# anhtu293/nndepth

Hardware: AMD Instinct MI355X
Metric: stereo pairs/sec at 544x960, 32 iters (RAFT-Stereo) (higher is better)
Workload: dtype f32 carried as 2 range-scaled fp16 pieces per operand (3 MFMA products, fp32 accumulate)

## Files before the change

### nndepth_amd/csrc/common.h

```cpp
#pragma once
#include <hip/hip_runtime.h>
#include <atomic>
#include <cstdarg>
#include <cstdio>
#include "../../include/nndepth_amd.h"

namespace nnd {

void set_error(const char* fmt, ...);

#define NND_HIP_CHECK(expr)                                                              \
    do {                                                                                 \
        hipError_t _e = (expr);                                                          \
        if (_e != hipSuccess) {                                                          \
            nnd::set_error("%s failed: %s (%s:%d)", #expr, hipGetErrorString(_e), __FILE__, __LINE__); \
            return NND_ERR_HIP;                                                          \
        }                                                                                \
    } while (0)

#define NND_LAUNCH_CHECK()                                                               \
    do {                                                                                 \
        hipError_t _e = hipGetLastError();                                               \
        if (_e != hipSuccess) {                                                          \
            nnd::set_error("kernel launch failed: %s (%s:%d)", hipGetErrorString(_e), __FILE__, __LINE__); \
            return NND_ERR_HIP;                                                          \
        }                                                                                \
    } while (0)

#define NND_REQUIRE(cond, ...)                                                           \
    do {                                                                                 \
        if (!(cond)) {                                                                   \
            nnd::set_error(__VA_ARGS__);                                                 \
            return NND_ERR_INVALID;                                                      \
        }                                                                                \
    } while (0)

struct Switches {
    bool no_fused_upsample, no_fused_lookup, no_fused_flow_branch, no_c4, agcl_v1, no_thin3d, corr_build_v1, corr_build_no_ksplit, igev_squeeze_v1, igev_squeeze_walk, no_folded_flow_head, no_conv1x1_stream,
        conv_verbose, debug_sync;
    int split_ny, split_ks, split_p;
    bool split_no_fast;
    bool no_merged_fb_lookup;
    int conv_p, conv_ks, conv_wco;
    int agcl_pb;
    bool lds_poison_on;
    unsigned lds_poison;
    int lds_slack;
    bool enc_no_c4;
    bool no_slab3d;
    int slab3d_rounds;
};
const Switches& switches();

static inline int raise_lds_limit(const void* kern, std::atomic<unsigned>& done, int bytes = 160 * 1024) {
    int dev = 0;
    NND_HIP_CHECK(hipGetDevice(&dev));
    const unsigned bit = 1u << (dev & 31);
    if (!(done.load(std::memory_order_relaxed) & bit)) {
        NND_HIP_CHECK(hipFuncSetAttribute(kern, hipFuncAttributeMaxDynamicSharedMemorySize, bytes));
        done.fetch_or(bit, std::memory_order_relaxed);
    }
    return NND_OK;
}

bool calibrating();
struct CalibScope {
    explicit CalibScope(bool on);
// ... 115 lines not shown
int lookup_convc1_launch(const float* pyr, const float* geo, int G, const float* coords, const ConvLayer& L, const float* blob,
                         float* c1, int64_t c1_bs, int B, int H, int W, int num_levels, int radius, hipStream_t stream, bool c1_c4);
bool flow_branch_lookup_supported(int arith);
int flow_branch_lookup_launch(const ConvLayer& f2, const float* blob, const float* w7t, const float* b7, const float* flow, int64_t fbs,
                              int fc, const ConvIO& io, const float* pyr, const float* coords, const ConvLayer& Lc1, float* c1,
                              int64_t c1_bs, int B, int H, int W, int num_levels, int radius, hipStream_t stream, bool c1_c4);
bool igev_lookup_convc1_il_supported(int G, int num_levels, int radius);
int igev_lookup_convc1_il_launch(const float* il, int G, const float* coords, const ConvLayer& L, const float* blob, float* c1,
                                 int64_t c1_bs, int B, int H, int W, int num_levels, int radius, hipStream_t stream, bool c1_c4);
struct MaskUpFlowHead {
    const float* x;
    long xbs;
    int hid;
    const float* w;
    const float* bias;
    const float* coords_in;
    float *coords_out, *flow_out, *delta_out;
    float* hx_flow;
    long hx_bs;
    int hx_pm;
    int absolute;
};

bool mask_upsample_supported(int rate, int cin, int flow_channels);
bool mask_upsample_fold_supported(const ConvLayer& L, int hid);
int mask_upsample_launch(const ConvLayer& L, const float* blob, const float* x, int64_t xbs, const float* flow, float* out,
                         int B, int H, int W, int rate, hipStream_t stream, bool tiled, int flow_channels = 1, bool x_c4 = false,
                         const MaskUpFlowHead* fh = nullptr);

}
```

### nndepth_amd/csrc/error.cpp

```cpp
#include "common.h"

#include <cstdlib>

namespace nnd {
static thread_local char g_err[512] = "";
void set_error(const char* fmt, ...) {
    va_list ap;
    va_start(ap, fmt);
    vsnprintf(g_err, sizeof(g_err), fmt, ap);
    va_end(ap);
}

static Switches g_sw;
static void load_switches() {
    Switches s{};
    auto on = [](const char* n) { return getenv(n) != nullptr; };
    s.no_fused_upsample = on("NND_NO_FUSED_UPSAMPLE");
    s.no_fused_lookup = on("NND_NO_FUSED_LOOKUP");
    s.no_fused_flow_branch = on("NND_NO_FUSED_FLOW_BRANCH");
    s.no_c4 = on("NND_NO_C4");
    s.agcl_v1 = on("NND_AGCL_V1");
    s.no_thin3d = on("NND_NO_THIN3D");
    s.corr_build_v1 = on("NND_CORR_BUILD_V1");
    s.corr_build_no_ksplit = on("NND_CORR_BUILD_NO_KSPLIT");
    s.igev_squeeze_v1 = on("NND_IGEV_SQUEEZE_V1");
    s.igev_squeeze_walk = on("NND_IGEV_SQUEEZE_WALK");
    s.no_folded_flow_head = on("NND_NO_FOLDED_FLOW_HEAD");
    s.no_conv1x1_stream = on("NND_NO_CONV1X1_STREAM");
    s.conv_verbose = on("NND_CONV_VERBOSE");
    s.debug_sync = on("NND_DEBUG_SYNC");
    s.split_ny = s.split_ks = s.split_p = -1;
    if (const char* e = getenv("NND_SPLIT_CFG")) sscanf(e, "%d,%d,%d", &s.split_ny, &s.split_ks, &s.split_p);
    s.split_no_fast = on("NND_SPLIT_NO_FAST");
    s.no_merged_fb_lookup = on("NND_NO_MERGED_FB_LOOKUP");
    s.conv_p = s.conv_ks = s.conv_wco = -1;
    if (const char* e = getenv("NND_CONV_CFG")) sscanf(e, "%d,%d,%d", &s.conv_p, &s.conv_ks, &s.conv_wco);
    if (const char* e = getenv("NND_CONV_P")) s.conv_p = atoi(e);
    s.agcl_pb = getenv("NND_AGCL_PB") ? atoi(getenv("NND_AGCL_PB")) : 0;
    s.lds_poison_on = on("NND_DEBUG_LDS_POISON");
    s.lds_poison = s.lds_poison_on ? (unsigned)strtoul(getenv("NND_DEBUG_LDS_POISON"), nullptr, 0) : 0u;
    s.lds_slack = getenv("NND_DEBUG_LDS_SLACK") ? atoi(getenv("NND_DEBUG_LDS_SLACK")) : 0;
    s.enc_no_c4 = on("NND_ENC_NO_C4");
    s.no_slab3d = on("NND_NO_SLAB3D");
    s.slab3d_rounds = getenv("NND_SLAB3D_ROUNDS") ? atoi(getenv("NND_SLAB3D_ROUNDS")) : 0;
    g_sw = s;
}
namespace {
struct SwitchInit {
    SwitchInit() { load_switches(); }
} g_switch_init;
// ... 21 lines not shown
```

### nndepth_amd/csrc/mask_upsample.hip

```cpp
#include "common.h"

#include <type_traits>
#include "layout.h"
#include "split_arith.h"

namespace nnd {

typedef float f32x16 __attribute__((ext_vector_type(16)));

#ifdef NND_DBG_STAMPS
__device__ unsigned long long g_mu_stamps[4096 * 8];
#define NND_MSTAMP(i)                                                                             \
    do {                                                                                          \
        if (threadIdx.x == 0 && blockIdx.x < 4096) g_mu_stamps[blockIdx.x * 8 + (i)] = __builtin_amdgcn_s_memrealtime(); \
    } while (0)
#else
#define NND_MSTAMP(i)
#endif

struct MaskUpArgs {
    const float* x;
    long xbs;
    const float* wpk;
    const float* bias;
    const float* flow;
    float* out;
    int H, W, tiles_x, fc;
    Lay lay;
    int x_c4;
    int lds_floats;
    MaskUpFlowHead fh;
};

template <int RATE, int CIN>
struct MaskUpCfg {
    static constexpr int COUT = 9 * RATE * RATE;
    static constexpr int NCB = (COUT + 31) / 32;
    static constexpr int CBW = NCB >= 12 ? 3 : 1;
    static constexpr int G = (NCB + CBW - 1) / CBW;
    static constexpr int NWAVES = 2 * G;
    static constexpr int NT = 64 * NWAVES;
    static constexpr int NST = CIN / 32;
    static constexpr int MT_STRIDE = 33;
    static constexpr int XS_FLOATS = CIN * 32 * 3 / 2;
    static constexpr int LDS_FLOATS = (XS_FLOATS > COUT * MT_STRIDE ? XS_FLOATS : COUT * MT_STRIDE) + 128;
};

template <int RATE, int CIN, int NS = 0, int FHW = 0>
__global__ void __launch_bounds__((MaskUpCfg<RATE, CIN>::NT + 64 * FHW)) mask_upsample_kernel(MaskUpArgs a) {
    constexpr bool SPLIT = NS != 0;
    using Cfg = MaskUpCfg<RATE, CIN>;
    constexpr int COUT = Cfg::COUT, NCB = Cfg::NCB, CBW = Cfg::CBW, G = Cfg::G, NT = Cfg::NT, NST = Cfg::NST;
    constexpr int CI_T = 128;
    constexpr int NCHUNK = CIN / CI_T;
    constexpr int MTS = Cfg::MT_STRIDE;
    static_assert(CIN % 128 == 0 && NST % 2 == 0, "CIN must be a multiple of 128");
    extern __shared__ float lds[];
    NND_MSTAMP(0);
    float* xs = lds;
    float* mt = lds;
    float* fp = lds + a.lds_floats - 128;

    const int tid = threadIdx.x, lane = tid & 63;
    const int wave = __builtin_amdgcn_readfirstlane(tid >> 6);
    const int g = wave % G, kj = wave / G;
    const int h2 = lane >> 5, l31 = lane & 31;
    const int tx0 = (blockIdx.x % a.tiles_x) * 8, ty0 = (blockIdx.x / a.tiles_x) * 4;
    const int b = blockIdx.z;
    const int H = a.H, W = a.W;
    const long HW = (long)H * W;
    const long XP = a.lay.plane;
    float oscale = 1.f, xscale = 1.f;
    if constexpr (NS == 2) {
        oscale = a.bias[Cfg::NCB * 32 + SPLIT_TAIL_OSCALE];
        xscale = a.bias[Cfg::NCB * 32 + SPLIT_TAIL_XSCALE];
    }

    float fh_state = 0.f, fh_bias = 0.f;
    auto fh_finish = [&](float* fbase, int t0) {
        if (t0 >= 60) return;
        const float* part = fbase + a.fh.hid * 105;
        const int pr = t0 / 10, pc = t0 % 10;
        const int y = ty0 + pr - 1, x = tx0 + pc - 1;
        float sum = 0.f;
#pragma unroll
        for (int sl = 0; sl < 16; ++sl) sum += part[sl * 64 + t0];
        sum += fh_bias;
        const bool in = y >= 0 && y < H && x >= 0 && x < W;
        const float cnew = fh_state + sum;
        const float fl = a.fh.absolute ? cnew : cnew - (float)x;
        fp[t0] = in ? fl : 0.f;
        if (in && pr >= 1 && pr <= 4 && pc >= 1 && pc <= 8) {
            const long pix = pix_off(a.lay, y, x);
            a.fh.delta_out[b * XP + pix] = sum;
            a.fh.coords_out[b * XP + pix] = cnew;
            a.fh.flow_out[b * XP + pix] = fl;
            a.fh.hx_flow[b * a.fh.hx_bs + pix * a.fh.hx_pm] = fl;
        }
    };
    constexpr int NQ4 = (CIN / 4 * 32 + NT - 1) / NT;
    float4 v4[SPLIT ? NQ4 : 1];
    if constexpr (SPLIT) {
        const float* src = a.x + b * a.xbs;
#pragma unroll
        for (int i = 0; i < NQ4; ++i) {
            const int e = min(tid, NT - 1) + i * NT;
            const int qd = e >> 5, px = e & 31;
            const int y = ty0 + (px >> 3), x = tx0 + (px & 7);
            const bool ok = e < CIN / 4 * 32 && y < H && x < W;
            if (a.x_c4) {
                v4[i] = *reinterpret_cast<const float4*>(src + (ok ? (unsigned)(qd * 4 * (int)XP + 4 * (int)pix_off(a.lay, y, x)) : 0u));
            } else {
                const unsigned o = ok ? (unsigned)(qd * 4 * (int)XP + (int)pix_off(a.lay, y, x)) : 0u;
                v4[i] = make_float4(src[o], src[ok ? o + (unsigned)XP : 0u], src[ok ? o + 2u * (unsigned)XP : 0u], src[ok ? o + 3u * (unsigned)XP : 0u]);
            }
        }
    }
    if constexpr (FHW > 0) {
        if (tid >= NT) {
            float* fbase = lds + Cfg::LDS_FLOATS;
            const int hid = a.fh.hid, fw_ = __builtin_amdgcn_readfirstlane((tid - NT) >> 6), cn = hid / FHW, c0 = fw_ * cn;
            float* patch = fbase;
            float* fw = fbase + hid * 96;
            const float* src = a.fh.x + b * a.fh.xbs;
            constexpr int NPL = 12, NWL = 5;
            const int total = 96 * (cn / 4), nwt = cn * 9;
            float4 pv[NPL];
            bool pok[NPL];
            float wreg[NWL];
#pragma unroll
            for (int k = 0; k < NWL; ++k) wreg[k] = a.fh.w[c0 * 9 + min(lane + 64 * k, nwt - 1)];
            if (tid - NT < 60) {
                fh_bias = a.fh.bias[0];
                const int y = ty0 + (tid - NT) / 10 - 1, x = tx0 + (tid - NT) % 10 - 1;
                if (y >= 0 && y < H && x >= 0 && x < W) fh_state = a.fh.coords_in[b * XP + pix_off(a.lay, y, x)];
            }
#pragma unroll
// ... 43 lines not shown
#pragma unroll
                        for (int t = 0; t < 9; ++t) wv[k][t] = wk[t];
                    }
#pragma unroll
                    for (int k = 0; k < 4; ++k)
#pragma unroll
                        for (int t = 0; t < 9; ++t) fmac_scalar(acc[k], wv[k][t], xv[k][t]);
                }
                float* part = fbase + hid * 105;
                if (lane < 60)
#pragma unroll
                    for (int k = 0; k < 4; ++k) part[(s0 + k) * 64 + pos] = acc[k];
            }
            __syncthreads();
            fh_finish(fbase, tid - NT);
            __syncthreads();
            __syncthreads();
            return;
        }
    }
    {
        const float* src = a.x + b * a.xbs;
        if constexpr (SPLIT) {
            unsigned char* xsb = reinterpret_cast<unsigned char*>(lds);
#pragma unroll
            for (int i = 0; i < NQ4; ++i) {
                const int e = tid + i * NT;
                const int qd = e >> 5, px = e & 31;
                const bool ok = (ty0 + (px >> 3)) < H && (tx0 + (px & 7)) < W;
                if (e < CIN / 4 * 32) {
                    const float res[4] = {ok ? v4[i].x : 0.f, ok ? v4[i].y : 0.f, ok ? v4[i].z : 0.f, ok ? v4[i].w : 0.f};
                    const int chunk = qd >> 2, sub = qd & 3;
                    constexpr int NP = NS == 0 ? 3 : NS;
                    uint2 pv[NP];
                    split_pieces_n<NP, 4, uint2>(res, pv, xscale);
#pragma unroll
                    for (int sp = 0; sp < NP; ++sp)
                        *reinterpret_cast<uint2*>(xsb + ((((chunk * NP + sp) * 2 + (sub >> 1)) * 32 + px) * 16 + (sub & 1) * 8)) = pv[sp];
                }
            }
        } else
        if (a.x_c4) {
            constexpr int NQ4 = (CIN / 4 * 32 + NT - 1) / NT;
            float4 v4[NQ4];
#pragma unroll
            for (int i = 0; i < NQ4; ++i) {
                const int e = tid + i * NT;
                const int qd = e >> 5, px = e & 31;
                const int y = ty0 + (px >> 3), x = tx0 + (px & 7);
                const bool ok = e < CIN / 4 * 32 && y < H && x < W;
                v4[i] = *reinterpret_cast<const float4*>(src + (ok ? (unsigned)(qd * 4 * (int)XP + 4 * (int)pix_off(a.lay, y, x)) : 0u));
            }
#pragma unroll
            for (int i = 0; i < NQ4; ++i) {
// ... 9 lines not shown
            }
        } else {
        constexpr int NLD = (CIN * 32 + NT - 1) / NT;
        float v[NLD];
#pragma unroll
        for (int i = 0; i < NLD; ++i) {
            const int e = tid + i * NT;
            const int ci = e >> 5, px = e & 31;
            const int y = ty0 + (px >> 3), x = tx0 + (px & 7);
            const bool ok = e < CIN * 32 && y < H && x < W;
            v[i] = src[ok ? (unsigned)(ci * (int)XP + (int)pix_off(a.lay, y, x)) : 0u];
        }
#pragma unroll
        for (int i = 0; i < NLD; ++i) {
            const int e = tid + i * NT;
            const int px = e & 31;
            const bool ok = (ty0 + (px >> 3)) < H && (tx0 + (px & 7)) < W;
            if (e < CIN * 32) xs[e] = ok ? v[i] : 0.f;
        }
        }
        if (!a.fh.x && tid < 60 * a.fc) {
            const int f = tid / 60, pos = tid % 60;
            const int pr = pos / 10, pc = pos % 10;
            const int y = ty0 + pr - 1, x = tx0 + pc - 1;
            fp[tid] = (y >= 0 && y < H && x >= 0 && x < W) ? a.flow[(b * a.fc + f) * XP + pix_off(a.lay, y, x)] : 0.f;
        }
    }
    __syncthreads();
    NND_MSTAMP(1);

    f32x16 acc[CBW];
#pragma unroll
    for (int i = 0; i < CBW; ++i)
#pragma unroll
        for (int r = 0; r < 16; ++r) acc[i][r] = 0.f;
    if constexpr (SPLIT) {
        constexpr int NP = NS == 0 ? 3 : NS;
        constexpr int NCH16 = CIN / 16, CPW = NCH16 / 2;
        const uint4* wq4 = reinterpret_cast<const uint4*>(a.wpk);
        const unsigned char* xsb = reinterpret_cast<const unsigned char*>(lds);
        const int c0k = kj * CPW;
        auto a_ptr = [&](int cbi, int ch) {
            int cb = g * CBW + cbi;
            cb = cb < NCB ? cb : NCB - 1;
            return wq4 + (size_t)((cb * NCH16 + c0k + ch) * NP) * 64 + lane;
        };
        constexpr int AD = 3, NA = AD + 1, NUNIT = CPW * CBW;
        uint4 ab[NA][NP], bq[2][NP];
        auto load_a = [&](uint4* dst, int u) {
            const uint4* w = a_ptr(u % CBW, u / CBW);
#pragma unroll
            for (int sp = 0; sp < NP; ++sp) dst[sp] = w[sp * 64];
        };
        auto load_b = [&](uint4* dst, int ch) {
#pragma unroll
            for (int sp = 0; sp < NP; ++sp)
                dst[sp] = *reinterpret_cast<const uint4*>(xsb + (((((c0k + ch) * NP + sp) * 2 + h2) * 32 + l31) * 16));
        };
#pragma unroll
        for (int u = 0; u < AD && u < NUNIT; ++u) load_a(ab[u], u);
        load_b(bq[0], 0);
#pragma unroll
        for (int u = 0; u < NUNIT; ++u) {
            const int ch = u / CBW, cbi = u % CBW;
            if (u + AD < NUNIT) load_a(ab[(u + AD) % NA], u + AD);
            if (cbi == 0 && ch + 1 < CPW) load_b(bq[(ch + 1) & 1], ch + 1);
            __builtin_amdgcn_sched_barrier(0);
            split_mfma_step<NP>(ab[u % NA], bq[ch & 1], acc[cbi]);
            __builtin_amdgcn_sched_barrier(0);
        }
        if constexpr (NS == 2) {
#pragma unroll
            for (int cbi = 0; cbi < CBW; ++cbi)
#pragma unroll
                for (int r = 0; r < 16; ++r) acc[cbi][r] *= oscale;
        }
    } else {
        constexpr int SPW = NST / 2;
        const int s0 = kj * SPW;
        const float4* wq = reinterpret_cast<const float4*>(a.wpk);
        auto a_base = [&](int cbi) {
            int cb = g * CBW + cbi;
            cb = cb < NCB ? cb : NCB - 1;
            return wq + (size_t)cb * (NCHUNK * 16 * 64);
        };
        float4 ab[2][4];
        float bq[2][16];
        auto load_a = [&](float4* dst, int u) {
            const int s = s0 + u / CBW, cbi = u % CBW;
            const float4* ws = a_base(cbi) + s * (4 * 64);
    #pragma unroll
            for (int q = 0; q < 4; ++q) dst[q] = ws[(unsigned)(q * 64 + lane)];
        };
        auto load_b = [&](float* dst, int sl) {
            const float* xb = xs + ((s0 + sl) * 32 + h2) * 32 + l31;
    #pragma unroll
            for (int pair = 0; pair < 16; ++pair) dst[pair] = xb[pair * 64];
        };
        load_a(ab[0], 0);
        load_b(bq[0], 0);
    #pragma unroll
        for (int u = 0; u < SPW * CBW; ++u) {
            const int sl = u / CBW, cbi = u % CBW;
            if (u + 1 < SPW * CBW) load_a(ab[(u + 1) & 1], u + 1);
            if (cbi == 0 && sl + 1 < SPW) load_b(bq[(sl + 1) & 1], sl + 1);
            __builtin_amdgcn_sched_barrier(0);
    #pragma unroll
            for (int pair = 0; pair < 16; ++pair) {
                const float4 av = ab[u & 1][pair / 4];
                const float as = (pair % 4 == 0) ? av.x : (pair % 4 == 1) ? av.y : (pair % 4 == 2) ? av.z : av.w;
                acc[cbi] = __builtin_amdgcn_mfma_f32_32x32x2f32(as, bq[sl & 1][pair], acc[cbi], 0, 0, 0);
            }
            __builtin_amdgcn_sched_barrier(0);
        }
}
    NND_MSTAMP(2);
    __syncthreads();

#pragma unroll
    for (int pass = 0; pass < 2; ++pass) {
        if (kj == pass) {
#pragma unroll
            for (int cbi = 0; cbi < CBW; ++cbi) {
                const int cb = g * CBW + cbi;
#pragma unroll
                for (int reg = 0; reg < 16; ++reg) {
                    const int co = cb * 32 + (reg & 3) + 8 * (reg >> 2) + 4 * h2;
                    if (cb < NCB && co < COUT) {
                        float* p = mt + co * MTS + l31;
                        *p = pass == 0 ? acc[cbi][reg] : *p + acc[cbi][reg];
                    }
                }
            }
        }
        __syncthreads();
    }

    NND_MSTAMP(3);
    constexpr int ROWLEN = 8 * RATE;
    constexpr int NITEM = 4 * RATE * ROWLEN;
    const long OW = (long)W * RATE;
    for (int e = tid; e < NITEM; e += NT) {
        const int seg = e / ROWLEN, within = e % ROWLEN;
        const int rr = seg / RATE, i = seg % RATE;
        const int c = within / RATE, j = within % RATE;
        const int px = rr * 8 + c;
        const int y = ty0 + rr, x = tx0 + c;
        float m[9];
        float mx = -INFINITY;
#pragma unroll
        for (int k = 0; k < 9; ++k) {
            const int co = k * RATE * RATE + i * RATE + j;
            m[k] = 0.25f * (mt[co * MTS + px] + a.bias[co]);
            mx = fmaxf(mx, m[k]);
        }
        float sum = 0.f;
#pragma unroll
        for (int k = 0; k < 9; ++k) {
            m[k] = expf(m[k] - mx);
            sum += m[k];
        }
#pragma unroll
        for (int k = 0; k < 9; ++k) m[k] = m[k] / sum;
        for (int f = 0; f < a.fc; ++f) {
            float o = 0.f;
#pragma unroll
            for (int k = 0; k < 9; ++k) o += m[k] * ((float)RATE * fp[f * 60 + (rr + k / 3) * 10 + c + k % 3]);
            if (y < H && x < W) a.out[((long)b * a.fc + f) * HW * RATE * RATE + ((long)y * RATE + i) * OW + (long)x * RATE + j] = o;
        }
    }
#ifdef NND_DBG_STAMPS
    __builtin_amdgcn_s_waitcnt(0);
#endif
    NND_MSTAMP(4);
}

constexpr int MU_FHW = 4;
template <int RATE, int CIN, int NS, int FHW>
static int launch_mu_fhw(MaskUpArgs a, int B, hipStream_t stream) {
    using Cfg = MaskUpCfg<RATE, CIN>;
    auto kern = mask_upsample_kernel<RATE, CIN, NS, FHW>;
    a.lds_floats = Cfg::LDS_FLOATS;
    const int fh_floats = a.fh.x ? a.fh.hid * (96 + 9) + 16 * 64 : 0;
    if (FHW > 0) a.lds_floats = Cfg::LDS_FLOATS + fh_floats + 128;
    const size_t lds = a.lds_floats * sizeof(float);
    if (lds > 64 * 1024) {
        static std::atomic<unsigned> raised{0};
        if (int rc = raise_lds_limit(reinterpret_cast<const void*>(kern), raised)) return rc;
    }
    dim3 grid(a.tiles_x * cdiv(a.H, 4), 1, B), block(Cfg::NT + 64 * FHW);
    hipLaunchKernelGGL(kern, grid, block, lds, stream, a);
    NND_LAUNCH_CHECK();
    return NND_OK;
}
template <int RATE, int CIN, int NS = 0>
static int launch_mu(const MaskUpArgs& a, int B, hipStream_t stream) {
    if (a.fh.x) {
        if constexpr (NS == 2) return launch_mu_fhw<RATE, CIN, NS, MU_FHW>(a, B, stream);
        else NND_REQUIRE(false, "mask_upsample: the folded flow head is built for the fp16x2 arithmetic");
    }
    return launch_mu_fhw<RATE, CIN, NS, 0>(a, B, stream);
}

bool mask_upsample_fold_supported(const ConvLayer& L, int hid) { return L.arith == 2 && hid % 16 == 0 && hid <= 128; }

bool mask_upsample_supported(int rate, int cin, int flow_channels) {
    return (flow_channels == 1 || flow_channels == 2) && ((rate == 8 && (cin == 256 || cin == 128)) || (rate == 4 && (cin == 256 || cin == 128)));
}

int mask_upsample_launch(const ConvLayer& L, const float* blob, const float* x, int64_t xbs, const float* flow, float* out,
                         int B, int H, int W, int rate, hipStream_t stream, bool tiled, int flow_channels, bool x_c4,
                         const MaskUpFlowHead* fh) {
    NND_REQUIRE(L.KH == 1 && L.KW == 1 && L.CI_T == (L.arith ? 16 : 128) && L.Cout == 9 * rate * rate && (L.arith == 0 || L.arith == 3 || L.arith == 2),
                "mask_upsample: layer shape / packing");
    NND_REQUIRE(mask_upsample_supported(rate, L.Cin, flow_channels), "mask_upsample: rate %d / Cin %d / %d flow channels not built",
                rate, L.Cin, flow_channels);
    MaskUpArgs a;
    a.x = x; a.xbs = xbs; a.wpk = blob + L.w_off; a.bias = blob + L.b_off; a.flow = flow; a.out = out;
    a.H = H; a.W = W; a.tiles_x = cdiv(W, 8); a.fc = flow_channels;
    a.lay = make_lay(H, W, tiled);
    a.x_c4 = (tiled && x_c4) ? 1 : 0;
    a.lds_floats = 0;
    a.fh = MaskUpFlowHead{};
    if (fh && fh->x) {
        NND_REQUIRE(flow_channels == 1 && mask_upsample_fold_supported(L, fh->hid) && fh->w && fh->bias && fh->coords_in && fh->coords_out && fh->flow_out &&
                        fh->delta_out && fh->hx_flow && fh->coords_in != fh->coords_out,
                    "mask_upsample: folded flow head needs one flow channel, hid %% 16 == 0 and distinct old / new state buffers");
        a.fh = *fh;
    }
    if (L.arith == 3) {
        if (rate == 8 && L.Cin == 256) return launch_mu<8, 256, 3>(a, B, stream);
        if (rate == 8 && L.Cin == 128) return launch_mu<8, 128, 3>(a, B, stream);
        if (rate == 4 && L.Cin == 256) return launch_mu<4, 256, 3>(a, B, stream);
        return launch_mu<4, 128, 3>(a, B, stream);
    }
    if (L.arith == 2) {
        if (calibrating()) {
            const Act xa{const_cast<float*>(x), xbs, L.Cin};
            if (int rc = calib_amax_act(xa, make_lay(H, W, tiled, x_c4), B, H, W, blob + L.tail_off(), stream)) return rc;
        }
        if (rate == 8 && L.Cin == 256) return launch_mu<8, 256, 2>(a, B, stream);
        if (rate == 8 && L.Cin == 128) return launch_mu<8, 128, 2>(a, B, stream);
        if (rate == 4 && L.Cin == 256) return launch_mu<4, 256, 2>(a, B, stream);
        return launch_mu<4, 128, 2>(a, B, stream);
    }
    if (rate == 8 && L.Cin == 256) return launch_mu<8, 256>(a, B, stream);
    if (rate == 8 && L.Cin == 128) return launch_mu<8, 128>(a, B, stream);
    if (rate == 4 && L.Cin == 256) return launch_mu<4, 256>(a, B, stream);
    return launch_mu<4, 128>(a, B, stream);
}

#ifdef NND_DBG_STAMPS
extern "C" int nnd_debug_read_mu_stamps(unsigned long long* host, int n) {
    return hipMemcpyFromSymbol(host, HIP_SYMBOL(g_mu_stamps), sizeof(unsigned long long) * n) == hipSuccess ? 0 : -1;
}
#endif

}
```

### nndepth_amd/csrc/update_block.hip

```cpp
#include "common.h"
#include "layout.h"

#include <cstdlib>
#include <cstring>
#include <vector>

namespace nnd {

enum ConvId { C_C1 = 0, C_C2, C_F2, C_CV, C_ZR1X, C_Q1X, C_ZR2X, C_Q2X, C_FHM, C_M2, C_LOOP_COUNT,
              C_ZR1 = C_LOOP_COUNT, C_Q1, C_ZR2, C_Q2, C_ZR1C, C_Q1C, C_ZR2C, C_Q2C, C_COUNT };
static const char* kConvNames[C_COUNT] = {"encoder.convc1", "encoder.convc2", "encoder.convf2", "encoder.conv",
                                          "gru.convz1+convr1[h,motion]", "gru.convq1[rh,motion]", "gru.convz2+convr2[h,motion]",
                                          "gru.convq2[rh,motion]", "flow_head.conv1+mask.0", "mask.2",
                                          "gru.convz1+convr1", "gru.convq1", "gru.convz2+convr2", "gru.convq2",
                                          "gru.convz1+convr1[inp]", "gru.convq1[inp]", "gru.convz2+convr2[inp]", "gru.convq2[inp]"};

struct Plan {
    nnd_update_block_desc d;
    bool sep;
    ConvLayer L[C_COUNT];
    int64_t f1_w, f1_b;
    int64_t f1_wt;
    int64_t fc2_w, fc2_b;
    int64_t total;
};
// ... 48 lines not shown
        p->L[zr - C_ZR1 + C_ZR1C] = mk(kh, kw, ctx, 2 * hid, &off, ar(zr - C_ZR1 + C_ZR1C));
        p->L[q - C_ZR1 + C_ZR1C] = mk(kh, kw, ctx, hid, &off, ar(q - C_ZR1 + C_ZR1C));
    }
    if (!p->sep)
        for (int base : {(int)C_ZR1X, (int)C_ZR1, (int)C_ZR1C}) {
            p->L[base + 2] = p->L[base];
            p->L[base + 3] = p->L[base + 1];
        }
    p->L[C_FHM] = mk(3, 3, hid, 3 * hid, &off, ar(C_FHM));
    p->fc2_w = off; off += (int64_t)fc * hid * 9;
    p->fc2_b = off; off += 4;
    p->L[C_M2] = mk(1, 1, 2 * hid, mc, &off, ar(C_M2));
    p->total = off;
    return NND_OK;
}

static int refuse_last_only(const nnd_update_block_desc* d, const char* what) {
    NND_REQUIRE(!d || !(d->flags & NND_FLAG_LAST_UPSAMPLE_ONLY), "%s: NND_FLAG_LAST_UPSAMPLE_ONLY applies to the refine entry points only", what);
    return NND_OK;
}

struct Bufs {
    float *c1, *cf, *f1, *hx, *z, *rh, *fm, *corr, *mask, *delta, *coords, *flow, *ctxb;
    int64_t total;
};

static void carve(const Plan& p, int B, int H, int W, float* base, Bufs* b) {
    const int64_t n = (int64_t)B * tiled_plane(H, W);
    const int hid = p.d.hidden_dim, ctx = p.d.context_dim, fc = p.d.flow_channels;
    int64_t off = 0;
    auto take = [&](int C) {
        float* ptr = base ? base + off : nullptr;
        off += ((int64_t)C * n + 63) / 64 * 64;
        return ptr;
    };
    b->c1 = take(256);
    b->cf = take(256);
    b->f1 = take(128);
    b->hx = take(2 * hid + ctx);
    b->z = take(hid);
    b->rh = take(hid);
    b->fm = take(3 * hid);
    b->corr = take(p.d.cor_planes);
    b->mask = take(p.d.mask_channels);
    b->delta = take(fc);
    b->coords = take(1);
    b->flow = take(fc);
    b->ctxb = take(6 * hid);
    b->total = off;
}

template <int FC>
__global__ void __launch_bounds__(256) convf1_kernel(const float* __restrict__ flow, long fbs, const float* __restrict__ w,
                                                     const float* __restrict__ bias, float* __restrict__ out, long obs,
                                                     int H, int W, int tiles_x, Lay lay) {
    __shared__ float patch[FC][14][40];
    __shared__ __attribute__((aligned(16))) float wl[16 * (FC * 49 + 3)];
    constexpr int WS = FC * 49 + 3;
    const int tid = threadIdx.x;
    const int tx0 = (blockIdx.x % tiles_x) * 32, ty0 = (blockIdx.x / tiles_x) * 8;
    const int b = blockIdx.z, co0 = blockIdx.y * 16;
    const long HW = lay.plane;
    for (int e = tid; e < FC * 14 * 38; e += 256) {
        int c = e / (14 * 38), rem = e % (14 * 38);
        int pr = rem / 38, pc = rem % 38;
        int gy = ty0 + pr - 3, gx = tx0 + pc - 3;
        patch[c][pr][pc] = (gy >= 0 && gy < H && gx >= 0 && gx < W) ? flow[b * fbs + c * HW + pix_off(lay, gy, gx)] : 0.f;
    }
    for (int e = tid; e < 16 * FC * 49; e += 256) wl[(e / (FC * 49)) * WS + e % (FC * 49)] = w[(long)co0 * (FC * 49) + e];
    __syncthreads();
    const int st = tid >> 5, within = tid & 31;
// ... 598 lines not shown
                        agcl_offset_cl_supported(cre->C) && !switches().agcl_v1;
    if (cre_cl) {
        NND_TRY(nchw_to_nhwc_launch(cre->f1, cre->warped, B, cre->C, H * W, s));
        NND_TRY(nchw_to_nhwc_launch(cre->f2, cre->warped + (int64_t)B * cre->C * H * W, B, cre->C, H * W, s));
    }
    Act c = act(w.corr, p.d.cor_planes * n, p.d.cor_planes);
    auto lookup = [&](hipStream_t st_, int it) -> int {
        if (cre) {
            if (cre->extra && cre_cl)
                return agcl_offset_cl_launch(cre->warped, cre->warped + (int64_t)B * cre->C * H * W, w.flow, cre->extra, w.corr, B, cre->C,
                                             H, W, it & 1, st_, true);
            if (cre->extra) return agcl_offset_launch(cre->f1, cre->f2, w.flow, cre->extra, w.corr, B, cre->C, H, W, it & 1, st_, true);
            return agcl_iter_launch(cre->f1, cre->f2, w.flow, cre->warped, w.corr, B, cre->C, H, W, it & 1, st_, true);
        }
        if (igev) return igev_lookup_launch(pyramid, geo_pyramid, w.coords, w.corr, B, groups, H, W, num_levels, radius, st_, true);
        if (flat_groups > 0) return group_lookup_flat_launch(pyramid, w.coords, w.corr, B, flat_groups, H, W, num_levels, radius, st_, true);
        return corr1d_lookup_launch(pyramid, w.coords, w.corr, B, H, W, num_levels, radius, st_, true);
    };
    for (int id : {(int)C_ZR1C, (int)C_Q1C, (int)C_ZR2C, (int)C_Q2C})
        if (p.sep || id < C_ZR2C) NND_TRY(run_conv(p, packed, w, id, c, nullptr, nullptr, B, H, W, s));
    const bool no_fuse_up = switches().no_fused_upsample;
    const bool no_fuse_lk = switches().no_fused_lookup;
    const bool fused_up = !no_fuse_up && mask_upsample_supported(rate, 2 * hid, fc);
    const bool fold_fh = fused_up && !cre && fc == 1 && mask_upsample_fold_supported(p.L[C_M2], hid) &&
                         (long)B * cdiv(H, 4) * cdiv(W, 8) <= 256 && !switches().no_folded_flow_head;
    float* coords_alt = w.mask;
    float* flow_alt = w.mask + ((int64_t)B * n + 63) / 64 * 64;
    const bool fused_lk = !cre && !no_fuse_lk && flat_groups == 0;
    const bool merged_fbl = fused_lk && !igev && !switches().no_merged_fb_lookup && !switches().no_fused_flow_branch &&
                            flow_branch_supported(p.L[C_F2], fc) && flow_branch_lookup_supported(p.L[C_F2].arith);
    auto loop_conv = [&](int id) -> int {
        probe_mark(id, s);
        const int rc_ = run_conv(p, packed, w, id, c, nullptr, nullptr, B, H, W, s);
        probe_mark(id, s);
        return rc_;
    };
    if (calibrating() && fused_lk && interleaved && p.L[C_C1].arith == 2 && igev_lookup_convc1_il_supported(groups, num_levels, radius))
        NND_TRY(calib_amax_flat(interleaved, nnd_igev_interleaved_floats(B, groups, H, W, num_levels), packed + p.L[C_C1].tail_off(), s));
    for (int it = 0; it < iters; ++it) {
        if (merged_fbl) {
            probe_mark(C_F2, s);
            NND_TRY(calib_flow_branch(p, packed, w, w.flow, B, H, W, s));
            const ConvIO fio = conv_io(p, w, C_F2, c, n, nullptr, nullptr);
            NND_TRY(flow_branch_lookup_launch(p.L[C_F2], packed, packed + p.f1_wt, packed + p.f1_b, w.flow, (int64_t)fc * n, fc, fio, pyramid,
                                              w.coords, p.L[C_C1], w.c1, 256 * n, B, H, W, num_levels, radius, s, ws_c4()));
            NND_TRY(debug_sync("encoder.convf1+convf2 | lookup+convc1", s));
            probe_mark(C_F2, s);
        } else {
// ... 10 lines not shown
            NND_TRY(debug_sync("lookup+convc1", s));
        } else {
            NND_TRY(lookup(s, it));
            NND_TRY(debug_sync("lookup", s));
            NND_TRY(run_conv(p, packed, w, C_C1, c, nullptr, nullptr, B, H, W, s));
        }
        }
        NND_TRY(loop_conv(C_C2));
        NND_TRY(loop_conv(C_CV));
        NND_TRY(loop_conv(C_ZR1X));
        NND_TRY(loop_conv(C_Q1X));
        if (p.sep) {
            NND_TRY(loop_conv(C_ZR2X));
            NND_TRY(loop_conv(C_Q2X));
        }
        if (last_only && it + 1 < iters) {
            ConvIO io = conv_io(p, w, C_FHM, c, n, nullptr, nullptr);
            io.cout_need = hid;
            NND_TRY(launch_conv(p.L[C_FHM], packed, io, conv_epi(C_FHM), B, H, W, s));
            NND_TRY(debug_sync("flow_head.conv1", s));
            NND_TRY(run_fc2(p, packed, w, w.delta, cre ? 2 : 1, igev, B, H, W, s));
            continue;
        }
        NND_TRY(loop_conv(C_FHM));
        float* up_it = up_out + (int64_t)it * up_iter_stride;
        if (fold_fh) {
            MaskUpFlowHead fh;
            fh.x = w.fm; fh.xbs = (int64_t)3 * hid * n; fh.hid = hid;
            fh.w = packed + p.fc2_w; fh.bias = packed + p.fc2_b;
            fh.coords_in = w.coords; fh.coords_out = coords_alt; fh.flow_out = flow_alt; fh.delta_out = w.delta;
            fh.hx_flow = hx_flow; fh.hx_bs = (long)(hxC * n); fh.hx_pm = ws_pm(); fh.absolute = igev ? 1 : 0;
            NND_TRY(mask_upsample_launch(p.L[C_M2], packed, w.fm + hid * n, (int64_t)3 * hid * n, w.flow, up_it, B, H, W, rate, s,
                                         true, fc, ws_c4(), &fh));
            NND_TRY(debug_sync("flow_head.conv2 + mask.2 + upsample", s));
            std::swap(w.coords, coords_alt);
            std::swap(w.flow, flow_alt);
            continue;
        }
        NND_TRY(run_fc2(p, packed, w, w.delta, cre ? 2 : 1, igev, B, H, W, s));
        if (fused_up) {
            NND_TRY(mask_upsample_launch(p.L[C_M2], packed, w.fm + hid * n, (int64_t)3 * hid * n, w.flow, up_it, B, H, W, rate, s,
                                         true, fc, ws_c4()));
            NND_TRY(debug_sync("mask.2 + upsample", s));
        } else {
            NND_TRY(run_conv(p, packed, w, C_M2, c, w.mask, nullptr, B, H, W, s));
            NND_TRY(convex_upsample_launch(w.flow, w.mask, up_it, B, fc, H, W, rate, s, true));
            NND_TRY(debug_sync("convex upsample", s));
        }
// ... 345 lines not shown
```

Baseline: 148.2.

## Defer mask upsampling and batch several iterations into one launch

Keeps a ring of per-iteration hidden-state and flow buffers and launches the convex mask upsample once per group of iterations, covering all grouped slots in one grid. It also lets one workgroup process two tiles so each weight load feeds MFMAs for both. This targets the small, poorly occupied per-iteration upsample launch at low resolution and its serial spot on the update loop. In exchange it uses extra workspace, turns off the folded flow-head path, and raises LDS and register use per workgroup.

After: 147.5. Within noise of the previous version (-0.5%).

```diff
diff --git a/nndepth_amd/csrc/common.h b/nndepth_amd/csrc/common.h
--- a/nndepth_amd/csrc/common.h
+++ b/nndepth_amd/csrc/common.h
@@ -36,13 +36,14 @@
     } while (0)
 
 struct Switches {
-    bool no_fused_upsample, no_fused_lookup, no_fused_flow_branch, no_c4, agcl_v1, no_thin3d, corr_build_v1, corr_build_no_ksplit, igev_squeeze_v1, igev_squeeze_walk, no_folded_flow_head, no_conv1x1_stream,
+    bool no_fused_upsample, no_fused_lookup, no_fused_flow_branch, no_c4, agcl_v1, no_thin3d, corr_build_v1, corr_build_no_ksplit, igev_squeeze_v1, igev_squeeze_walk, no_folded_flow_head, no_deferred_upsample, no_conv1x1_stream,
         conv_verbose, debug_sync;
     int split_ny, split_ks, split_p;
     bool split_no_fast;
     bool no_merged_fb_lookup;
     int conv_p, conv_ks, conv_wco;
     int agcl_pb;
+    int defer_g, defer_t;
     bool lds_poison_on;
     unsigned lds_poison;
     int lds_slack;
@@ -204,10 +205,17 @@
     int absolute;
 };
 
+struct MaskUpBatch {
+    int slots;
+    int64_t x_ss, flow_ss, out_ss;
+    int tiles_per_wg;
+};
+
 bool mask_upsample_supported(int rate, int cin, int flow_channels);
 bool mask_upsample_fold_supported(const ConvLayer& L, int hid);
+int mask_upsample_batch_tiles(const ConvLayer& L);
 int mask_upsample_launch(const ConvLayer& L, const float* blob, const float* x, int64_t xbs, const float* flow, float* out,
                          int B, int H, int W, int rate, hipStream_t stream, bool tiled, int flow_channels = 1, bool x_c4 = false,
-                         const MaskUpFlowHead* fh = nullptr);
+                         const MaskUpFlowHead* fh = nullptr, const MaskUpBatch* mb = nullptr);
 
 }
diff --git a/nndepth_amd/csrc/error.cpp b/nndepth_amd/csrc/error.cpp
--- a/nndepth_amd/csrc/error.cpp
+++ b/nndepth_amd/csrc/error.cpp
@@ -26,6 +26,9 @@
     s.igev_squeeze_v1 = on("NND_IGEV_SQUEEZE_V1");
     s.igev_squeeze_walk = on("NND_IGEV_SQUEEZE_WALK");
     s.no_folded_flow_head = on("NND_NO_FOLDED_FLOW_HEAD");
+    s.no_deferred_upsample = on("NND_NO_DEFERRED_UPSAMPLE");
+    s.defer_g = s.defer_t = -1;
+    if (const char* e = getenv("NND_DEFERRED_UPSAMPLE_CFG")) sscanf(e, "%d,%d", &s.defer_g, &s.defer_t);
     s.no_conv1x1_stream = on("NND_NO_CONV1X1_STREAM");
     s.conv_verbose = on("NND_CONV_VERBOSE");
     s.debug_sync = on("NND_DEBUG_SYNC");
diff --git a/nndepth_amd/csrc/mask_upsample.hip b/nndepth_amd/csrc/mask_upsample.hip
--- a/nndepth_amd/csrc/mask_upsample.hip
+++ b/nndepth_amd/csrc/mask_upsample.hip
@@ -26,13 +26,15 @@
     const float* flow;
     float* out;
     int H, W, tiles_x, fc;
+    int ntiles, nb;
+    long x_ss, flow_ss, out_ss;
     Lay lay;
     int x_c4;
     int lds_floats;
     MaskUpFlowHead fh;
 };
 
-template <int RATE, int CIN>
+template <int RATE, int CIN, int T = 1>
 struct MaskUpCfg {
     static constexpr int COUT = 9 * RATE * RATE;
     static constexpr int NCB = (COUT + 31) / 32;
@@ -43,13 +45,15 @@
     static constexpr int NST = CIN / 32;
     static constexpr int MT_STRIDE = 33;
     static constexpr int XS_FLOATS = CIN * 32 * 3 / 2;
-    static constexpr int LDS_FLOATS = (XS_FLOATS > COUT * MT_STRIDE ? XS_FLOATS : COUT * MT_STRIDE) + 128;
+    static constexpr int MT_FLOATS = COUT * MT_STRIDE;
+    static constexpr int LDS_FLOATS = T * ((XS_FLOATS > MT_FLOATS ? XS_FLOATS : MT_FLOATS) + 128);
 };
 
-template <int RATE, int CIN, int NS = 0, int FHW = 0>
+template <int RATE, int CIN, int NS = 0, int FHW = 0, int T = 1>
 __global__ void __launch_bounds__((MaskUpCfg<RATE, CIN>::NT + 64 * FHW)) mask_upsample_kernel(MaskUpArgs a) {
     constexpr bool SPLIT = NS != 0;
-    using Cfg = MaskUpCfg<RATE, CIN>;
+    using Cfg = MaskUpCfg<RATE, CIN, T>;
+    static_assert(T == 1 || (SPLIT && FHW == 0), "several tiles per workgroup: split arithmetics, no folded flow head");
     constexpr int COUT = Cfg::COUT, NCB = Cfg::NCB, CBW = Cfg::CBW, G = Cfg::G, NT = Cfg::NT, NST = Cfg::NST;
     constexpr int CI_T = 128;
     constexpr int NCHUNK = CIN / CI_T;
@@ -59,15 +63,25 @@
     NND_MSTAMP(0);
     float* xs = lds;
     float* mt = lds;
-    float* fp = lds + a.lds_floats - 128;
+    float* fp = lds + a.lds_floats - 128 * T;
 
     const int tid = threadIdx.x, lane = tid & 63;
     const int wave = __builtin_amdgcn_readfirstlane(tid >> 6);
     const int g = wave % G, kj = wave / G;
     const int h2 = lane >> 5, l31 = lane & 31;
-    const int tx0 = (blockIdx.x % a.tiles_x) * 8, ty0 = (blockIdx.x / a.tiles_x) * 4;
-    const int b = blockIdx.z;
     const int H = a.H, W = a.W;
+    int tx0s[T], ty0s[T];
+#pragma unroll
+    for (int t = 0; t < T; ++t) {
+        const int tile = blockIdx.x * T + t;
+        tx0s[t] = (tile % a.tiles_x) * 8;
+        ty0s[t] = tile < a.ntiles ? (tile / a.tiles_x) * 4 : H + 4;
+    }
+    const int tx0 = tx0s[0], ty0 = ty0s[0];
+    const int slot = blockIdx.z / a.nb, b = blockIdx.z % a.nb;
+    a.x += slot * a.x_ss;
+    a.flow += slot * a.flow_ss;
+    a.out += slot * a.out_ss;
     const long HW = (long)H * W;
     const long XP = a.lay.plane;
     float oscale = 1.f, xscale = 1.f;
@@ -99,20 +113,22 @@
         }
     };
     constexpr int NQ4 = (CIN / 4 * 32 + NT - 1) / NT;
-    float4 v4[SPLIT ? NQ4 : 1];
+    float4 v4[SPLIT ? T : 1][SPLIT ? NQ4 : 1];
     if constexpr (SPLIT) {
         const float* src = a.x + b * a.xbs;
+#pragma unroll
+        for (int t = 0; t < T; ++t)
 #pragma unroll
         for (int i = 0; i < NQ4; ++i) {
             const int e = min(tid, NT - 1) + i * NT;
             const int qd = e >> 5, px = e & 31;
-            const int y = ty0 + (px >> 3), x = tx0 + (px & 7);
+            const int y = ty0s[t] + (px >> 3), x = tx0s[t] + (px & 7);
             const bool ok = e < CIN / 4 * 32 && y < H && x < W;
             if (a.x_c4) {
-                v4[i] = *reinterpret_cast<const float4*>(src + (ok ? (unsigned)(qd * 4 * (int)XP + 4 * (int)pix_off(a.lay, y, x)) : 0u));
+                v4[t][i] = *reinterpret_cast<const float4*>(src + (ok ? (unsigned)(qd * 4 * (int)XP + 4 * (int)pix_off(a.lay, y, x)) : 0u));
             } else {
                 const unsigned o = ok ? (unsigned)(qd * 4 * (int)XP + (int)pix_off(a.lay, y, x)) : 0u;
-                v4[i] = make_float4(src[o], src[ok ? o + (unsigned)XP : 0u], src[ok ? o + 2u * (unsigned)XP : 0u], src[ok ? o + 3u * (unsigned)XP : 0u]);
+                v4[t][i] = make_float4(src[o], src[ok ? o + (unsigned)XP : 0u], src[ok ? o + 2u * (unsigned)XP : 0u], src[ok ? o + 3u * (unsigned)XP : 0u]);
             }
         }
     }
@@ -202,14 +218,16 @@
     {
         const float* src = a.x + b * a.xbs;
         if constexpr (SPLIT) {
-            unsigned char* xsb = reinterpret_cast<unsigned char*>(lds);
+#pragma unroll
+            for (int t = 0; t < T; ++t)
 #pragma unroll
             for (int i = 0; i < NQ4; ++i) {
+                unsigned char* xsb = reinterpret_cast<unsigned char*>(lds + t * Cfg::XS_FLOATS);
                 const int e = tid + i * NT;
                 const int qd = e >> 5, px = e & 31;
-                const bool ok = (ty0 + (px >> 3)) < H && (tx0 + (px & 7)) < W;
+                const bool ok = (ty0s[t] + (px >> 3)) < H && (tx0s[t] + (px & 7)) < W;
                 if (e < CIN / 4 * 32) {
-                    const float res[4] = {ok ? v4[i].x : 0.f, ok ? v4[i].y : 0.f, ok ? v4[i].z : 0.f, ok ? v4[i].w : 0.f};
+                    const float res[4] = {ok ? v4[t][i].x : 0.f, ok ? v4[t][i].y : 0.f, ok ? v4[t][i].z : 0.f, ok ? v4[t][i].w : 0.f};
                     const int chunk = qd >> 2, sub = qd & 3;
                     constexpr int NP = NS == 0 ? 3 : NS;
                     uint2 pv[NP];
@@ -265,18 +283,23 @@
         if (!a.fh.x && tid < 60 * a.fc) {
             const int f = tid / 60, pos = tid % 60;
             const int pr = pos / 10, pc = pos % 10;
-            const int y = ty0 + pr - 1, x = tx0 + pc - 1;
-            fp[tid] = (y >= 0 && y < H && x >= 0 && x < W) ? a.flow[(b * a.fc + f) * XP + pix_off(a.lay, y, x)] : 0.f;
+#pragma unroll
+            for (int t = 0; t < T; ++t) {
+                const int y = ty0s[t] + pr - 1, x = tx0s[t] + pc - 1;
+                fp[t * 128 + tid] = (y >= 0 && y < H && x >= 0 && x < W) ? a.flow[(b * a.fc + f) * XP + pix_off(a.lay, y, x)] : 0.f;
+            }
         }
     }
     __syncthreads();
     NND_MSTAMP(1);
 
-    f32x16 acc[CBW];
+    f32x16 acc[T][CBW];
+#pragma unroll
+    for (int t = 0; t < T; ++t)
 #pragma unroll
     for (int i = 0; i < CBW; ++i)
 #pragma unroll
-        for (int r = 0; r < 16; ++r) acc[i][r] = 0.f;
+        for (int r = 0; r < 16; ++r) acc[t][i][r] = 0.f;
     if constexpr (SPLIT) {
         constexpr int NP = NS == 0 ? 3 : NS;
         constexpr int NCH16 = CIN / 16, CPW = NCH16 / 2;
@@ -288,17 +311,19 @@
             cb = cb < NCB ? cb : NCB - 1;
             return wq4 + (size_t)((cb * NCH16 + c0k + ch) * NP) * 64 + lane;
         };
-        constexpr int AD = 3, NA = AD + 1, NUNIT = CPW * CBW;
-        uint4 ab[NA][NP], bq[2][NP];
+        constexpr int AD = T == 1 ? 3 : 2, NA = AD + 1, NUNIT = CPW * CBW;
+        uint4 ab[NA][NP], bq[2][T][NP];
         auto load_a = [&](uint4* dst, int u) {
             const uint4* w = a_ptr(u % CBW, u / CBW);
 #pragma unroll
             for (int sp = 0; sp < NP; ++sp) dst[sp] = w[sp * 64];
         };
-        auto load_b = [&](uint4* dst, int ch) {
+        auto load_b = [&](uint4 (*dst)[NP], int ch) {
+#pragma unroll
+            for (int t = 0; t < T; ++t)
 #pragma unroll
             for (int sp = 0; sp < NP; ++sp)
-                dst[sp] = *reinterpret_cast<const uint4*>(xsb + (((((c0k + ch) * NP + sp) * 2 + h2) * 32 + l31) * 16));
+                dst[t][sp] = *reinterpret_cast<const uint4*>(xsb + t * Cfg::XS_FLOATS * 4 + (((((c0k + ch) * NP + sp) * 2 + h2) * 32 + l31) * 16));
         };
 #pragma unroll
         for (int u = 0; u < AD && u < NUNIT; ++u) load_a(ab[u], u);
@@ -309,14 +334,17 @@
             if (u + AD < NUNIT) load_a(ab[(u + AD) % NA], u + AD);
             if (cbi == 0 && ch + 1 < CPW) load_b(bq[(ch + 1) & 1], ch + 1);
             __builtin_amdgcn_sched_barrier(0);
-            split_mfma_step<NP>(ab[u % NA], bq[ch & 1], acc[cbi]);
+#pragma unroll
+            for (int t = 0; t < T; ++t) split_mfma_step<NP>(ab[u % NA], bq[ch & 1][t], acc[t][cbi]);
             __builtin_amdgcn_sched_barrier(0);
         }
         if constexpr (NS == 2) {
 #pragma unroll
+            for (int t = 0; t < T; ++t)
+#pragma unroll
             for (int cbi = 0; cbi < CBW; ++cbi)
 #pragma unroll
-                for (int r = 0; r < 16; ++r) acc[cbi][r] *= oscale;
+                for (int r = 0; r < 16; ++r) acc[t][cbi][r] *= oscale;
         }
     } else {
         constexpr int SPW = NST / 2;
@@ -352,7 +380,7 @@
             for (int pair = 0; pair < 16; ++pair) {
                 const float4 av = ab[u & 1][pair / 4];
                 const float as = (pair % 4 == 0) ? av.x : (pair % 4 == 1) ? av.y : (pair % 4 == 2) ? av.z : av.w;
-                acc[cbi] = __builtin_amdgcn_mfma_f32_32x32x2f32(as, bq[sl & 1][pair], acc[cbi], 0, 0, 0);
+                acc[0][cbi] = __builtin_amdgcn_mfma_f32_32x32x2f32(as, bq[sl & 1][pair], acc[0][cbi], 0, 0, 0);
             }
             __builtin_amdgcn_sched_barrier(0);
         }
@@ -363,6 +391,8 @@
 #pragma unroll
     for (int pass = 0; pass < 2; ++pass) {
         if (kj == pass) {
+#pragma unroll
+            for (int t = 0; t < T; ++t)
 #pragma unroll
             for (int cbi = 0; cbi < CBW; ++cbi) {
                 const int cb = g * CBW + cbi;
@@ -370,8 +400,8 @@
                 for (int reg = 0; reg < 16; ++reg) {
                     const int co = cb * 32 + (reg & 3) + 8 * (reg >> 2) + 4 * h2;
                     if (cb < NCB && co < COUT) {
-                        float* p = mt + co * MTS + l31;
-                        *p = pass == 0 ? acc[cbi][reg] : *p + acc[cbi][reg];
+                        float* p = mt + t * Cfg::MT_FLOATS + co * MTS + l31;
+                        *p = pass == 0 ? acc[t][cbi][reg] : *p + acc[t][cbi][reg];
                     }
                 }
             }
@@ -383,7 +413,11 @@
     constexpr int ROWLEN = 8 * RATE;
     constexpr int NITEM = 4 * RATE * ROWLEN;
     const long OW = (long)W * RATE;
-    for (int e = tid; e < NITEM; e += NT) {
+    for (int et = tid; et < NITEM * T; et += NT) {
+        const int t = et / NITEM, e = et % NITEM;
+        const int tx0 = tx0s[t], ty0 = ty0s[t];
+        const float* mt_t = mt + t * Cfg::MT_FLOATS;
+        const float* fp_t = fp + t * 128;
         const int seg = e / ROWLEN, within = e % ROWLEN;
         const int rr = seg / RATE, i = seg % RATE;
         const int c = within / RATE, j = within % RATE;
@@ -394,7 +428,7 @@
 #pragma unroll
         for (int k = 0; k < 9; ++k) {
             const int co = k * RATE * RATE + i * RATE + j;
-            m[k] = 0.25f * (mt[co * MTS + px] + a.bias[co]);
+            m[k] = 0.25f * (mt_t[co * MTS + px] + a.bias[co]);
             mx = fmaxf(mx, m[k]);
         }
         float sum = 0.f;
@@ -408,7 +442,7 @@
         for (int f = 0; f < a.fc; ++f) {
             float o = 0.f;
 #pragma unroll
-            for (int k = 0; k < 9; ++k) o += m[k] * ((float)RATE * fp[f * 60 + (rr + k / 3) * 10 + c + k % 3]);
+            for (int k = 0; k < 9; ++k) o += m[k] * ((float)RATE * fp_t[f * 60 + (rr + k / 3) * 10 + c + k % 3]);
             if (y < H && x < W) a.out[((long)b * a.fc + f) * HW * RATE * RATE + ((long)y * RATE + i) * OW + (long)x * RATE + j] = o;
         }
     }
@@ -419,10 +453,10 @@
 }
 
 constexpr int MU_FHW = 4;
-template <int RATE, int CIN, int NS, int FHW>
+template <int RATE, int CIN, int NS, int FHW, int T = 1>
 static int launch_mu_fhw(MaskUpArgs a, int B, hipStream_t stream) {
-    using Cfg = MaskUpCfg<RATE, CIN>;
-    auto kern = mask_upsample_kernel<RATE, CIN, NS, FHW>;
+    using Cfg = MaskUpCfg<RATE, CIN, T>;
+    auto kern = mask_upsample_kernel<RATE, CIN, NS, FHW, T>;
     a.lds_floats = Cfg::LDS_FLOATS;
     const int fh_floats = a.fh.x ? a.fh.hid * (96 + 9) + 16 * 64 : 0;
     if (FHW > 0) a.lds_floats = Cfg::LDS_FLOATS + fh_floats + 128;
@@ -431,19 +465,25 @@
         static std::atomic<unsigned> raised{0};
         if (int rc = raise_lds_limit(reinterpret_cast<const void*>(kern), raised)) return rc;
     }
-    dim3 grid(a.tiles_x * cdiv(a.H, 4), 1, B), block(Cfg::NT + 64 * FHW);
+    dim3 grid(cdiv(a.ntiles, T), 1, B), block(Cfg::NT + 64 * FHW);
     hipLaunchKernelGGL(kern, grid, block, lds, stream, a);
     NND_LAUNCH_CHECK();
     return NND_OK;
 }
+constexpr int MU_BATCH_TILES = 2;
 template <int RATE, int CIN, int NS = 0>
-static int launch_mu(const MaskUpArgs& a, int B, hipStream_t stream) {
+static int launch_mu(const MaskUpArgs& a, int B, hipStream_t stream, int tiles_per_wg = 1) {
     if (a.fh.x) {
         if constexpr (NS == 2) return launch_mu_fhw<RATE, CIN, NS, MU_FHW>(a, B, stream);
         else NND_REQUIRE(false, "mask_upsample: the folded flow head is built for the fp16x2 arithmetic");
     }
+    if constexpr (NS == 2) {
+        if (tiles_per_wg == MU_BATCH_TILES) return launch_mu_fhw<RATE, CIN, NS, 0, MU_BATCH_TILES>(a, B, stream);
+    }
+    NND_REQUIRE(tiles_per_wg == 1, "mask_upsample: %d tiles per workgroup not built for this arithmetic", tiles_per_wg);
     return launch_mu_fhw<RATE, CIN, NS, 0>(a, B, stream);
 }
+int mask_upsample_batch_tiles(const ConvLayer& L) { return L.arith == 2 ? MU_BATCH_TILES : 1; }
 
 bool mask_upsample_fold_supported(const ConvLayer& L, int hid) { return L.arith == 2 && hid % 16 == 0 && hid <= 128; }
 
@@ -453,7 +493,7 @@
 
 int mask_upsample_launch(const ConvLayer& L, const float* blob, const float* x, int64_t xbs, const float* flow, float* out,
                          int B, int H, int W, int rate, hipStream_t stream, bool tiled, int flow_channels, bool x_c4,
-                         const MaskUpFlowHead* fh) {
+                         const MaskUpFlowHead* fh, const MaskUpBatch* mb) {
     NND_REQUIRE(L.KH == 1 && L.KW == 1 && L.CI_T == (L.arith ? 16 : 128) && L.Cout == 9 * rate * rate && (L.arith == 0 || L.arith == 3 || L.arith == 2),
                 "mask_upsample: layer shape / packing");
     NND_REQUIRE(mask_upsample_supported(rate, L.Cin, flow_channels), "mask_upsample: rate %d / Cin %d / %d flow channels not built",
@@ -465,6 +505,17 @@
     a.x_c4 = (tiled && x_c4) ? 1 : 0;
     a.lds_floats = 0;
     a.fh = MaskUpFlowHead{};
+    a.ntiles = a.tiles_x * cdiv(H, 4); a.nb = B;
+    a.x_ss = a.flow_ss = a.out_ss = 0;
+    int T = 1;
+    if (mb) {
+        NND_REQUIRE(mb->slots >= 1 && !(fh && fh->x) && !calibrating(), "mask_upsample: batched launch without folded flow head / calibration only");
+        NND_REQUIRE(mb->slots == 1 || mb->out_ss != 0, "mask_upsample: the slots of a batched launch need distinct outputs");
+        NND_REQUIRE((int64_t)mb->slots * B <= 65535, "mask_upsample: %d slots x batch %d exceed the grid", mb->slots, B);
+        a.x_ss = mb->x_ss; a.flow_ss = mb->flow_ss; a.out_ss = mb->out_ss;
+        T = mb->tiles_per_wg > 0 ? mb->tiles_per_wg : mask_upsample_batch_tiles(L);
+        B *= mb->slots;
+    }
     if (fh && fh->x) {
         NND_REQUIRE(flow_channels == 1 && mask_upsample_fold_supported(L, fh->hid) && fh->w && fh->bias && fh->coords_in && fh->coords_out && fh->flow_out &&
                         fh->delta_out && fh->hx_flow && fh->coords_in != fh->coords_out,
@@ -472,25 +523,25 @@
         a.fh = *fh;
     }
     if (L.arith == 3) {
-        if (rate == 8 && L.Cin == 256) return launch_mu<8, 256, 3>(a, B, stream);
-        if (rate == 8 && L.Cin == 128) return launch_mu<8, 128, 3>(a, B, stream);
-        if (rate == 4 && L.Cin == 256) return launch_mu<4, 256, 3>(a, B, stream);
-        return launch_mu<4, 128, 3>(a, B, stream);
+        if (rate == 8 && L.Cin == 256) return launch_mu<8, 256, 3>(a, B, stream, T);
+        if (rate == 8 && L.Cin == 128) return launch_mu<8, 128, 3>(a, B, stream, T);
+        if (rate == 4 && L.Cin == 256) return launch_mu<4, 256, 3>(a, B, stream, T);
+        return launch_mu<4, 128, 3>(a, B, stream, T);
     }
     if (L.arith == 2) {
         if (calibrating()) {
             const Act xa{const_cast<float*>(x), xbs, L.Cin};
             if (int rc = calib_amax_act(xa, make_lay(H, W, tiled, x_c4), B, H, W, blob + L.tail_off(), stream)) return rc;
         }
-        if (rate == 8 && L.Cin == 256) return launch_mu<8, 256, 2>(a, B, stream);
-        if (rate == 8 && L.Cin == 128) return launch_mu<8, 128, 2>(a, B, stream);
-        if (rate == 4 && L.Cin == 256) return launch_mu<4, 256, 2>(a, B, stream);
-        return launch_mu<4, 128, 2>(a, B, stream);
-    }
-    if (rate == 8 && L.Cin == 256) return launch_mu<8, 256>(a, B, stream);
-    if (rate == 8 && L.Cin == 128) return launch_mu<8, 128>(a, B, stream);
-    if (rate == 4 && L.Cin == 256) return launch_mu<4, 256>(a, B, stream);
-    return launch_mu<4, 128>(a, B, stream);
+        if (rate == 8 && L.Cin == 256) return launch_mu<8, 256, 2>(a, B, stream, T);
+        if (rate == 8 && L.Cin == 128) return launch_mu<8, 128, 2>(a, B, stream, T);
+        if (rate == 4 && L.Cin == 256) return launch_mu<4, 256, 2>(a, B, stream, T);
+        return launch_mu<4, 128, 2>(a, B, stream, T);
+    }
+    if (rate == 8 && L.Cin == 256) return launch_mu<8, 256>(a, B, stream, T);
+    if (rate == 8 && L.Cin == 128) return launch_mu<8, 128>(a, B, stream, T);
+    if (rate == 4 && L.Cin == 256) return launch_mu<4, 256>(a, B, stream, T);
+    return launch_mu<4, 128>(a, B, stream, T);
 }
 
 #ifdef NND_DBG_STAMPS
diff --git a/nndepth_amd/csrc/update_block.hip b/nndepth_amd/csrc/update_block.hip
--- a/nndepth_amd/csrc/update_block.hip
+++ b/nndepth_amd/csrc/update_block.hip
@@ -1,6 +1,7 @@
 #include "common.h"
 #include "layout.h"
 
+#include <algorithm>
 #include <cstdlib>
 #include <cstring>
 #include <vector>
@@ -95,8 +96,21 @@
 
 struct Bufs {
     float *c1, *cf, *f1, *hx, *z, *rh, *fm, *corr, *mask, *delta, *coords, *flow, *ctxb;
+    int ring;
+    int64_t fm_slot, flow_slot;
     int64_t total;
 };
+
+constexpr int DEFER_RING = 8;
+constexpr int DEFER_SLOTS = 8;
+static int mask_rate(const Plan& p) {
+    int r = 1;
+    while (9 * r * r < p.d.mask_channels) ++r;
+    return 9 * r * r == p.d.mask_channels ? r : 0;
+}
+static bool defer_shape(const Plan& p, int B, int H, int W) {
+    return p.d.flow_channels == 1 && mask_upsample_supported(mask_rate(p), 2 * p.d.hidden_dim, 1) && (long)B * cdiv(H, 4) * cdiv(W, 8) <= 256;
+}
 
 static void carve(const Plan& p, int B, int H, int W, float* base, Bufs* b) {
     const int64_t n = (int64_t)B * tiled_plane(H, W);
@@ -113,13 +127,20 @@
     b->hx = take(2 * hid + ctx);
     b->z = take(hid);
     b->rh = take(hid);
-    b->fm = take(3 * hid);
     b->corr = take(p.d.cor_planes);
     b->mask = take(p.d.mask_channels);
     b->delta = take(fc);
     b->coords = take(1);
+    b->ctxb = take(6 * hid);
+    b->ring = defer_shape(p, B, H, W) ? DEFER_RING : 0;
+    int64_t at = off;
     b->flow = take(fc);
-    b->ctxb = take(6 * hid);
+    b->flow_slot = off - at;
+    for (int k = 1; k < b->ring; ++k) take(fc);
+    at = off;
+    b->fm = take(3 * hid);
+    b->fm_slot = off - at;
+    for (int k = 1; k < b->ring; ++k) take(3 * hid);
     b->total = off;
 }
 
@@ -764,8 +785,14 @@
     const bool no_fuse_up = switches().no_fused_upsample;
     const bool no_fuse_lk = switches().no_fused_lookup;
     const bool fused_up = !no_fuse_up && mask_upsample_supported(rate, 2 * hid, fc);
+    const bool defer_up = fused_up && !cre && fc == 1 && !calibrating() && !last_flag && up_iter_stride != 0 && w.ring > 0 &&
+                          !switches().no_deferred_upsample;
+    const int defer_g = switches().defer_g > 0 ? std::min(switches().defer_g, w.ring) : DEFER_SLOTS;
+    const int defer_t = switches().defer_t > 0 ? switches().defer_t : 0;
+    float* const fm0 = w.fm;
+    float* const flow0 = w.flow;
     const bool fold_fh = fused_up && !cre && fc == 1 && mask_upsample_fold_supported(p.L[C_M2], hid) &&
-                         (long)B * cdiv(H, 4) * cdiv(W, 8) <= 256 && !switches().no_folded_flow_head;
+                         (long)B * cdiv(H, 4) * cdiv(W, 8) <= 256 && !switches().no_folded_flow_head && !defer_up;
     float* coords_alt = w.mask;
     float* flow_alt = w.mask + ((int64_t)B * n + 63) / 64 * 64;
     const bool fused_lk = !cre && !no_fuse_lk && flat_groups == 0;
@@ -822,8 +849,21 @@
             NND_TRY(run_fc2(p, packed, w, w.delta, cre ? 2 : 1, igev, B, H, W, s));
             continue;
         }
+        if (defer_up) w.fm = fm0 + (it % defer_g) * w.fm_slot;
         NND_TRY(loop_conv(C_FHM));
         float* up_it = up_out + (int64_t)it * up_iter_stride;
+        if (defer_up) {
+            const int slot = it % defer_g;
+            w.flow = flow0 + slot * w.flow_slot;
+            NND_TRY(run_fc2(p, packed, w, w.delta, 1, igev, B, H, W, s));
+            if (slot == defer_g - 1 || it + 1 == iters) {
+                const MaskUpBatch mb{slot + 1, w.fm_slot, w.flow_slot, up_iter_stride, defer_t};
+                NND_TRY(mask_upsample_launch(p.L[C_M2], packed, fm0 + hid * n, (int64_t)3 * hid * n, flow0,
+                                             up_out + (int64_t)(it - slot) * up_iter_stride, B, H, W, rate, s, true, fc, ws_c4(), nullptr, &mb));
+                NND_TRY(debug_sync("mask.2 + upsample (batched)", s));
+            }
+            continue;
+        }
         if (fold_fh) {
             MaskUpFlowHead fh;
             fh.x = w.fm; fh.xbs = (int64_t)3 * hid * n; fh.hid = hid;
```
